# Wendison/FCL-taco2

Hardware: AMD Instinct MI355X
Metric: mel-frames/sec (FCL-taco2-S forward, batch=32, 80-mel) (higher is better)
Workload: dtype f32 via bf16x3-split MFMA operands, fp32 accumulate (max-abs 8e-6 on mel vs the reference; FCL_PRECISION=0 = exact fp32 MFMA)

## Files before the change

### fcl-taco2_amd/csrc/capi.hip

```cpp
#include <stdarg.h>
#include <stdlib.h>
#include <string.h>

#include <map>
#include <mutex>
#include <utility>
#include <vector>

#include "fcl_common.h"

namespace fcl {

static thread_local char g_err[512] = "";
static thread_local int g_gemm_mode = FCL_GEMM_F32;

void set_error(const char* fmt, ...) {
    va_list ap;
    va_start(ap, fmt);
    vsnprintf(g_err, sizeof(g_err), fmt, ap);
    va_end(ap);
}

int check_hip(hipError_t e, const char* what) {
    static const int sync_debug = getenv("FCL_SYNC_DEBUG") ? atoi(getenv("FCL_SYNC_DEBUG")) : 0;
// ... 474 lines not shown
    FCL_REQUIRE(io->dropout_mode != FCL_DROP_MASK || io->prenet_keep, FCL_ERR_INVALID, "decoder_loop_fwd: FCL_DROP_MASK needs prenet_keep");
    FCL_REQUIRE(w->prenet_dropout >= 0.f && w->prenet_dropout < 1.f, FCL_ERR_INVALID, "decoder_loop_fwd: bad prenet_dropout");
    FCL_REQUIRE(io->workspace && aligned16(io->workspace) && io->workspace_bytes >= fcl_decoder_loop_workspace_bytes(w, io->n), FCL_ERR_WORKSPACE,
                "decoder_loop_fwd: workspace missing, misaligned or smaller than fcl_decoder_loop_workspace_bytes()");
    FCL_REQUIRE(!io->live_rows || io->status, FCL_ERR_INVALID, "decoder_loop_fwd: device live_rows need a device status word");
    {
        int prev = io->n;
        FCL_REQUIRE(io->live_rows || io->live_rows_host[0] == io->n, FCL_ERR_INVALID, "decoder_loop_fwd: live_rows_host[0] must equal N (all durations > 0)");
        for (int t = 0; t < io->lmax; ++t) {
            FCL_REQUIRE(io->live_rows_host[t] > 0 && io->live_rows_host[t] <= prev, FCL_ERR_INVALID,
                        "decoder_loop_fwd: live_rows_host must be positive and non-increasing (rows sorted by duration descending)");
            prev = io->live_rows_host[t];
        }
    }
    hipStream_t s = (hipStream_t)stream;
    if (generic) return decoder_loop_generic(w, io, s);
    const int N = io->n, C = w->c, P = w->p, U = w->u, O = w->odim;
    DecoderWs ws = carve(w, N, io->workspace);

    static const bool planes_on = tunable("PRECISION", 1) != 0 && tunable("PLANES", 1) != 0;
    const bool planes = decoder_planes(w) && io->att_c_p != nullptr && planes_on;
    FCL_REQUIRE(planes || io->att_c, FCL_ERR_INVALID, "decoder_loop_fwd: att_c is required when the P32 path is off");
    FCL_REQUIRE(!io->before_p || planes, FCL_ERR_INVALID, "decoder_loop_fwd: before_p needs the P32 weight planes and att_c_p");
    {
        hipLaunchKernelGGL(zero_kernel, dim3(512), dim3(256), 0, s, ws.h0[0], (long long)(ws.state_bytes / 4));
        FCL_HIP(hipGetLastError());
    }
    const int ldc = C / 32, ldp = P / 32, ldu = U / 32;
    auto small_step = [&](int m) { return lstm_step_is_small(m, U); };
    {
        GemmArgs g = {};
        g.term[0] = GemmTerm{io->att_c, w->w0_att, C, C, C, 0};
        if (planes) { g.term[0].Ap = io->att_c_p; g.term[0].Wp = w->w0_att_p; g.term[0].lda_p = g.term[0].ldw_p = ldc; }
        g.nterms = 1; g.M = N; g.N = 4 * U; g.bias = w->b0; g.Y = ws.G0; g.ldy = 4 * U;
        int rc = launch_gemm(g, s);
        if (rc) return rc;
        GemmArgs f = {};
        f.term[0] = GemmTerm{io->att_c, w->wf_att, C, C, C, 0};
        if (planes) { f.term[0].Ap = io->att_c_p; f.term[0].Wp = w->wf_att_p; f.term[0].lda_p = f.term[0].ldw_p = ldc; }
        f.nterms = 1; f.M = N; f.N = O; f.Y = ws.F0; f.ldy = O;
        rc = launch_gemm(f, s);
        if (rc) return rc;
    }
    const float keep_scale = 1.0f / (1.0f - w->prenet_dropout);
    const int drop_mode = (w->prenet_dropout > 0.f) ? io->dropout_mode : FCL_DROP_NONE;
    {
        static const int tile_on = tunable("DEC_TILE", 0), tile_min = tunable("DEC_TILE_MIN_ROWS", 1024);
        if (tile_on && planes && w->stream && decoder_tile_shape_ok(w) && N >= tile_min && io->lmax <= 64 && !io->teacher_ys && !io->tap_prenet && !io->tap_lstm0 &&
            !io->tap_lstm1 && drop_mode != FCL_DROP_MASK && gemm_mode() != FCL_GEMM_BF16)
            return launch_decoder_tile(w, io, ws.G0, ws.F0, ws.c0, ws.c1, drop_mode, 0, nullptr, nullptr, s);
    }
    const bool tile_ok = planes && w->stream && decoder_tile_shape_ok(w) && io->lmax <= 64 && !io->teacher_ys && !io->tap_prenet && !io->tap_lstm0 && !io->tap_lstm1 &&
                         drop_mode != FCL_DROP_MASK && gemm_mode() != FCL_GEMM_BF16;
    const int tail_from = (tile_ok && io->tail_from > 0 && io->tail_from < io->lmax) ? io->tail_from : 0;
    int cur = 0;
    for (int t = 0; t <= io->lmax; ++t) {
        const bool hand_over = tail_from > 0 && t == tail_from;
        const int n = (t < io->lmax && !hand_over) ? io->live_rows_host[t] : 0;
        const int n_prev = t > 0 ? io->live_rows_host[t - 1] : 0;
        const uint8_t* keep0 = drop_mode == FCL_DROP_MASK && t < io->lmax ? io->prenet_keep + ((size_t)(t * 2 + 0) * N) * P : nullptr;
        const uint8_t* keep1 = drop_mode == FCL_DROP_MASK && t < io->lmax ? io->prenet_keep + ((size_t)(t * 2 + 1) * N) * P : nullptr;
        const unsigned seed0 = io->seed * 2654435761u + (unsigned)(t * 2 + 0), seed1 = seed0 + 1;
        const float* teacher_in = (io->teacher_ys && t > 0) ? io->teacher_ys + (size_t)(t - 1) * O : nullptr;
        FeatPrenetArgs fp = {};
        fp.M_feat = n_prev; fp.M_pre = n; fp.U = U; fp.O = O; fp.P = P;
        fp.h1 = t > 0 ? ws.h1[cur] : nullptr; fp.wf_h = w->wf_h; fp.F0 = ws.F0;
        fp.before = io->before; fp.frame_off = io->frame_off; fp.t_prev = t - 1; fp.t_cur = t;
        fp.teacher_in = teacher_in; fp.teacher_ld = io->lmax * O;
        if (t < io->lmax && !hand_over) { fp.w0 = w->prenet_w0; fp.b0 = w->prenet_b0; fp.w1 = w->prenet_w1; fp.b1 = w->prenet_b1; }
        fp.wf_hi = w->wf_h_hi; fp.wf_lo = w->wf_h_lo; fp.w0_hi = w->prenet_w0_hi; fp.w0_lo = w->prenet_w0_lo;
        fp.w1_hi = w->prenet_w1_hi; fp.w1_lo = w->prenet_w1_lo;
        fp.wf_ff = w->wf_h_ff; fp.w0_ff = w->prenet_w0_ff; fp.w1_ff = w->prenet_w1_ff;
        fp.drop_mode = drop_mode; fp.keep0 = keep0; fp.keep1 = keep1; fp.keep_scale = keep_scale; fp.drop_p = w->prenet_dropout;
        fp.seed0 = seed0; fp.seed1 = seed1; fp.seed_dev = io->seed_dev; fp.pre_out = ws.pre_b; fp.tap_prenet = io->tap_prenet;
        fp.live = io->live_rows; fp.status = io->status; fp.out_act = w->out_act;
        if (planes) {
            fp.before_p = io->before_p;
            if (!small_step(n)) { fp.pre_out_p = ws.pre_p; fp.pre_out = nullptr; }
        }
        int rc = launch_feat_prenet(fp, s);
        if (rc) return rc;
        if (hand_over) return launch_decoder_tile(w, io, ws.G0, ws.F0, ws.c0, ws.c1, drop_mode, t, ws.h0[cur], ws.h1[cur], s);
        if (t == io->lmax) break;
        LstmStepArgs l0 = {};
        const bool big = planes && !small_step(n);
        const bool next_big = planes && t + 1 < io->lmax && !small_step(io->live_rows_host[t + 1]);
        l0.term[0] = GemmTerm{ws.pre_b, w->w0_pre, P, P, P, 0, w->w0_pre_hi, w->w0_pre_lo};
        l0.term[1] = GemmTerm{ws.h0[cur], w->w0_hh, U, U, U, 0, w->w0_hh_hi, w->w0_hh_lo};
        if (big) {
            l0.term[0].Ap = ws.pre_p; l0.term[0].Wp = w->w0_pre_p; l0.term[0].lda_p = l0.term[0].ldw_p = ldp;
            l0.term[1].Ap = ws.h0_p[cur]; l0.term[1].Wp = w->w0_hh_p; l0.term[1].lda_p = l0.term[1].ldw_p = ldu;
            l0.h_out_p = ws.h0_p[cur ^ 1]; l0.ld_hp = ldu;
        }
        l0.term[0].Wff = w->w0_pre_ff; l0.term[1].Wff = w->w0_hh_ff;
        l0.nterms = 2; l0.M = n; l0.U = U; l0.G = ws.G0; l0.g_row_mul = 1; l0.g_row_add = 0;
        l0.m_dev = io->live_rows ? io->live_rows + t : nullptr;
        l0.rank1_w = w->w0_pos; l0.dur = io->dur; l0.step = t;
        l0.h_in = ws.h0[cur]; l0.h_out = ws.h0[cur ^ 1]; l0.c = ws.c0; l0.zoneout = w->zoneout_rate;
        if (io->tap_lstm0) { l0.out2 = io->tap_lstm0; l0.out2_row_base = io->frame_off; l0.out2_row_add = t; l0.ld2 = U; }
        rc = launch_lstm_step(l0, s);
        if (rc) return rc;
        LstmStepArgs l1 = {};
        l1.term[0] = GemmTerm{ws.h0[cur ^ 1], w->w1_ih, U, U, U, 0, w->w1_ih_hi, w->w1_ih_lo};
        l1.term[1] = GemmTerm{ws.h1[cur], w->w1_hh, U, U, U, 0, w->w1_hh_hi, w->w1_hh_lo};
        if (big) {
            l1.term[0].Ap = ws.h0_p[cur ^ 1]; l1.term[0].Wp = w->w1_ih_p; l1.term[0].lda_p = l1.term[0].ldw_p = ldu;
            l1.term[1].Ap = ws.h1_p[cur]; l1.term[1].Wp = w->w1_hh_p; l1.term[1].lda_p = l1.term[1].ldw_p = ldu;
            if (next_big) { l1.h_out_p = ws.h1_p[cur ^ 1]; l1.ld_hp = ldu; }
        }
        l1.term[0].Wff = w->w1_ih_ff; l1.term[1].Wff = w->w1_hh_ff;
        l1.nterms = 2; l1.M = n; l1.U = U; l1.bias = w->b1; l1.step = t;
        l1.m_dev = l0.m_dev;
        l1.h_in = ws.h1[cur]; l1.h_out = ws.h1[cur ^ 1]; l1.c = ws.c1; l1.zoneout = w->zoneout_rate;
        if (io->tap_lstm1) { l1.out2 = io->tap_lstm1; l1.out2_row_base = io->frame_off; l1.out2_row_add = t; l1.ld2 = U; }
        rc = launch_lstm_step(l1, s);
        if (rc) return rc;
        cur ^= 1;
    }
    return 0;
}

}
```

### fcl-taco2_amd/csrc/decoder_step.hip

```cpp
#include "fcl_common.h"
#include "lstm_epilogue.h"

namespace fcl {

typedef float f32x4 __attribute__((ext_vector_type(4)));

template <int NT>
__device__ __forceinline__ void rowtile_mma(const float* A_l, int lda_l, const float* const (&wrow)[NT], int K, int r16, int kq,
                                            f32x4 (&out)[NT], int rot = 0) {
    f32x4 acc0[NT], acc1[NT];
#pragma unroll
    for (int t = 0; t < NT; ++t) acc0[t] = acc1[t] = (f32x4){0.f, 0.f, 0.f, 0.f};
    const float* ap = A_l + r16 * lda_l + kq * 4;
    const float* wp[NT];
#pragma unroll
    for (int t = 0; t < NT; ++t) wp[t] = wrow[t] + kq * 4;
    const int nfull = K >> 6;
    f32x4 bn[NT][4];
    int cc = nfull > 0 ? rot % nfull : 0;
    if (nfull > 0) {
#pragma unroll
        for (int t = 0; t < NT; ++t)
#pragma unroll
            for (int i = 0; i < 4; ++i) bn[t][i] = *reinterpret_cast<const f32x4*>(wp[t] + (cc << 6) + i * 16);
// ... 848 lines not shown
        }
    }
}

template <bool PRE>
__global__ __launch_bounds__(256) void lstm_small_x3_kernel(const LstmStepArgs a) {
    const int M = a.M, Ms = live_rows_of(a.M, a.m_dev);
    if ((int)blockIdx.y * 16 >= Ms) return;
    constexpr int KC = 512;
    __shared__ __attribute__((aligned(16))) u16 A_h[16 * (KC + 16)];
    __shared__ __attribute__((aligned(16))) u16 A_lo[16 * (KC + 16)];
    __shared__ float g_l[4][16][17];
    const int m0 = blockIdx.y * 16, u0 = blockIdx.x * 16;
    const int lane = threadIdx.x & 63, g = threadIdx.x >> 6;
    const int r16 = lane & 15, kq = lane >> 4;
    const int erow = threadIdx.x >> 4, euc = threadIdx.x & 15;
    const int em = m0 + erow, eu = u0 + euc;
    const bool evalid = em < M && eu < a.U;
    CellIn ci;
    if (evalid) ci = cell_prefetch(a, em, eu);
    f32x4 acc = {0.f, 0.f, 0.f, 0.f};
    WFrag<1, 8> wf[2];
    if (PRE) {
#pragma unroll
        for (int t = 0; t < 2; ++t) {
            const size_t fo = (size_t)((g * a.U + u0) >> 4) * 8 * 512 + (size_t)lane * 8;
            const u16* const wh[1] = {a.term[t].Whi + fo};
            const u16* const wl[1] = {a.term[t].Wlo + fo};
            wf[t].load(wh, wl);
        }
#pragma unroll
        for (int t = 0; t < 2; ++t) {
            if (t) __syncthreads();
            load_rowtile_split(A_h, A_lo, 256 + 16, a.term[t].A, a.term[t].lda, 256, m0, M);
            __syncthreads();
            f32x4 part[1];
            wf[t].mma(A_h, A_lo, 256 + 16, 256, r16, kq, part);
            acc += part[0];
        }
    }
    for (int t = 0; t < (PRE ? 0 : a.nterms); ++t) {
        const GemmTerm T = a.term[t];
        for (int k0 = 0; k0 < T.K; k0 += KC) {
            const int kc = min(KC, T.K - k0);
            __syncthreads();
            load_rowtile_split(A_h, A_lo, kc + 16, T.A + k0, T.lda, kc, m0, M);
            __syncthreads();
            const size_t fo = ((size_t)((g * a.U + u0) >> 4) * ((T.K + 31) >> 5) + (k0 >> 5)) * 512 + (size_t)lane * 8;
            const u16* const wh[1] = {T.Whi + fo};
            const u16* const wl[1] = {T.Wlo + fo};
            f32x4 part[1];
            rowtile_mma_x3<1>(A_h, A_lo, kc + 16, wh, wl, kc, r16, kq, part);
            acc += part[0];
        }
    }
// ... 5 lines not shown
    __syncthreads();
    if (!evalid || em >= Ms) return;
    const float pre[4] = {g_l[0][erow][euc], g_l[1][erow][euc], g_l[2][erow][euc], g_l[3][erow][euc]};
    cell_finish(a, em, eu, pre, ci);
}


__global__ __launch_bounds__(256) void lstm_small_ff_kernel(const LstmStepArgs a) {
    const int M = a.M, Ms = live_rows_of(a.M, a.m_dev);
    if ((int)blockIdx.y * 16 >= Ms) return;
    constexpr int LD = 256 + 8;
    __shared__ __attribute__((aligned(16))) float A_f[16 * LD];
    __shared__ float g_l[4][16][17];
    const int m0 = blockIdx.y * 16, u0 = blockIdx.x * 16;
    const int lane = threadIdx.x & 63, g = threadIdx.x >> 6;
    const int r16 = lane & 15, kq = lane >> 4;
    const int erow = threadIdx.x >> 4, euc = threadIdx.x & 15;
    const int em = m0 + erow, eu = u0 + euc;
    const bool evalid = em < M && eu < a.U;
    CellIn ci;
    if (evalid) ci = cell_prefetch(a, em, eu);
    f32x4 acc = {0.f, 0.f, 0.f, 0.f};
    WFragF<1, 8> wf[2];
#pragma unroll
    for (int t = 0; t < 2; ++t) {
        const float* const w[1] = {a.term[t].Wff + (size_t)((g * a.U + u0) >> 4) * 8 * 512 + (size_t)lane * 8};
        wf[t].load(w);
    }
#pragma unroll
    for (int t = 0; t < 2; ++t) {
        if (t) __syncthreads();
        load_rowtile(A_f, LD, a.term[t].A, a.term[t].lda, 256, m0, M);
        __syncthreads();
        f32x4 part[1];
        mma_tf<1, 8>(wf[t], A_f, LD, r16, kq, part);
        acc += part[0];
    }
    {
        const int arow = lane & 15, cq = lane >> 4;
#pragma unroll
        for (int i = 0; i < 4; ++i) g_l[g][arow][cq * 4 + i] = acc[i];
    }
    __syncthreads();
    if (!evalid || em >= Ms) return;
    const float pre[4] = {g_l[0][erow][euc], g_l[1][erow][euc], g_l[2][erow][euc], g_l[3][erow][euc]};
    cell_finish(a, em, eu, pre, ci);
}

constexpr int SMALL_KC = 512;

__device__ __forceinline__ void lstm_small_body(const LstmStepArgs& a) {
    const int M = a.M, Ms = live_rows_of(a.M, a.m_dev);
    if ((int)blockIdx.y * 16 >= Ms) return;
// ... 25 lines not shown
    __syncthreads();
    const int row = threadIdx.x >> 4, uc = threadIdx.x & 15;
    const int m = m0 + row, uu = u0 + uc;
    if (m >= Ms || uu >= a.U) return;
    const CellIn ci = cell_prefetch(a, m, uu);
    const float pre[4] = {g_l[0][row][uc], g_l[1][row][uc], g_l[2][row][uc], g_l[3][row][uc]};
    cell_finish(a, m, uu, pre, ci);
}

__global__ __launch_bounds__(256) void lstm_small_kernel(const LstmStepArgs a) { lstm_small_body(a); }

__global__ __launch_bounds__(256) void lstm_small_pair_kernel(const LstmStepArgs a0, const LstmStepArgs a1) {
    if (blockIdx.z == 0) lstm_small_body(a0);
    else lstm_small_body(a1);
}

int launch_lstm_small(const LstmStepArgs& a, hipStream_t s) {
    double ksum = 0;
    for (int i = 0; i < a.nterms; ++i) ksum += a.term[i].K;
    dim3 grid((a.U + 15) / 16, (a.M + 15) / 16);
    bool planes = true;
    for (int i = 0; i < a.nterms; ++i) planes = planes && a.term[i].Whi && a.term[i].Wlo && (a.term[i].K & 7) == 0 && a.term[i].ldw == a.term[i].K;
    planes = planes && (a.U & 15) == 0;
    if (planes) {
        ProfScope ps("lstm_small_kernel/bf16x3", 2.0 * a.M * 4.0 * a.U * ksum, a.M, s);
        if (a.nterms == 2 && a.term[0].K == 256 && a.term[1].K == 256) hipLaunchKernelGGL(lstm_small_x3_kernel<true>, grid, dim3(256), 0, s, a);
        else hipLaunchKernelGGL(lstm_small_x3_kernel<false>, grid, dim3(256), 0, s, a);
    } else if (a.nterms == 2 && a.term[0].Wff && a.term[1].Wff && a.term[0].K == 256 && a.term[1].K == 256 && (a.U & 15) == 0) {
        ProfScope ps("lstm_small_ff_kernel/f32", 2.0 * a.M * 4.0 * a.U * ksum, a.M, s);
        hipLaunchKernelGGL(lstm_small_ff_kernel, grid, dim3(256), 0, s, a);
    } else {
        ProfScope ps("lstm_small_kernel", 2.0 * a.M * 4.0 * a.U * ksum, a.M, s);
        hipLaunchKernelGGL(lstm_small_kernel, grid, dim3(256), 0, s, a);
    }
    return check_hip(hipGetLastError(), "lstm_small launch");
}

int launch_lstm_small_pair(const LstmStepArgs& a0, const LstmStepArgs& a1, hipStream_t s) {
    double fl = 0;
    for (const LstmStepArgs* a : {&a0, &a1}) {
        double ksum = 0;
        for (int i = 0; i < a->nterms; ++i) ksum += a->term[i].K;
        fl += 2.0 * a->M * 4.0 * a->U * ksum;
    }
    const int mmax = a0.M > a1.M ? a0.M : a1.M;
    dim3 grid((a0.U + 15) / 16, (mmax + 15) / 16, 2);
    ProfScope ps("lstm_small_pair_kernel", fl, a0.M + a1.M, s);
    hipLaunchKernelGGL(lstm_small_pair_kernel, grid, dim3(256), 0, s, a0, a1);
    return check_hip(hipGetLastError(), "lstm_small_pair launch");
}

// ... 79 lines not shown
```

### fcl-taco2_amd/csrc/gemm_f32.hip

```cpp
#include <string.h>

#include "fcl_common.h"
#include "lstm_epilogue.h"

namespace fcl {

typedef float f32x4 __attribute__((ext_vector_type(4)));

#ifndef FCL_BK
#define FCL_BK 32
#endif
constexpr int BK = FCL_BK;
constexpr int F4 = BK / 4;
constexpr int F4_SHIFT = F4 == 8 ? 3 : 2;
static_assert(BK == 32 || BK == 16, "BK must be 16 or 32");
#ifndef FCL_NBUF
#define FCL_NBUF 2
#endif
constexpr int NBUF = FCL_NBUF;
constexpr int LDS_LD = BK + 4;

template <int WM, int WN, bool LSTM, int TM = 1>
struct Geo {
    static constexpr int BM = 16 * WM * TM;
// ... 389 lines not shown
    using G = Geo<WM, WN, false, TM>;
    dim3 grid((a.N + G::BN - 1) / G::BN, (a.M + G::BM - 1) / G::BM);
    char full[64];
    GemmArgs b = a;
    b.hi_only = precision() && gemm_mode() == FCL_GEMM_BF16;
    snprintf(full, sizeof(full), "gemm_kernel<%d,%d,%d,%d>%s", WM, WN, precision() ? 1 : 0, TM, b.hi_only ? "/bf16" : precision() ? "/bf16x3" : "");
    static const int shapes = tunable("PROF_SHAPES", 0);
    if (shapes && g_prof_on) {
        long long ks = 0;
        for (int i = 0; i < a.nterms; ++i) ks += a.term[i].K;
        const size_t l = strlen(full);
        snprintf(full + l, sizeof(full) - l, " %dx%dx%lld", a.M, a.N, ks);
    }
    (void)name;
    ProfScope ps(full, flops, a.M, s);
    if (precision()) hipLaunchKernelGGL((gemm_kernel<WM, WN, 1, TM>), grid, dim3(G::THREADS), 0, s, b);
    else hipLaunchKernelGGL((gemm_kernel<WM, WN, 0, TM>), grid, dim3(G::THREADS), 0, s, b);
}

template <int WM, int WN, int TM = 1>
static void launch_lstm_cfg(const LstmStepArgs& a, hipStream_t s, const char* name, double flops) {
    using G = Geo<WM, WN, true, TM>;
    dim3 grid((a.U + 16 * WN - 1) / (16 * WN), (a.M + G::BM - 1) / G::BM);
    const bool plain = !a.zone_keep_h && !a.row_len;
    const int mode = (plain && a.G && a.rank1_w && !a.bias) ? 0 : (plain && a.bias && !a.G && !a.rank1_w) ? 1 : -1;
    char full[64];
    const int hi_only = precision() && gemm_mode() == FCL_GEMM_BF16;
    snprintf(full, sizeof(full), "lstm_step_kernel<%d,%d,%d,%d,%d>%s", WM, WN, mode, precision() ? 1 : 0, TM, hi_only ? "/bf16" : precision() ? "/bf16x3" : "");
    (void)name;
    ProfScope ps(full, flops, a.M, s);
    if (precision()) {
        if (mode == 0) hipLaunchKernelGGL((lstm_step_kernel<WM, WN, 0, 1, TM>), grid, dim3(G::THREADS), 0, s, a, hi_only);
        else if (mode == 1) hipLaunchKernelGGL((lstm_step_kernel<WM, WN, 1, 1, TM>), grid, dim3(G::THREADS), 0, s, a, hi_only);
        else hipLaunchKernelGGL((lstm_step_kernel<WM, WN, -1, 1, TM>), grid, dim3(G::THREADS), 0, s, a, hi_only);
    } else {
        if (mode == 0) hipLaunchKernelGGL((lstm_step_kernel<WM, WN, 0, 0, TM>), grid, dim3(G::THREADS), 0, s, a, hi_only);
        else if (mode == 1) hipLaunchKernelGGL((lstm_step_kernel<WM, WN, 1, 0, TM>), grid, dim3(G::THREADS), 0, s, a, hi_only);
        else hipLaunchKernelGGL((lstm_step_kernel<WM, WN, -1, 0, TM>), grid, dim3(G::THREADS), 0, s, a, hi_only);
    }
}

extern thread_local bool t_exact_lines;
static bool exact_lines_ok(const GemmTerm* t, int n) {
    if (precision()) return false;
    for (int i = 0; i < n; ++i) {
        if (!t[i].A || !t[i].W || (t[i].K & 31) || (t[i].lda & 31) || (t[i].ldw & 31) || t[i].lda < t[i].K || t[i].ldw < t[i].K || t[i].a_chunk_stride) return false;
        if ((reinterpret_cast<uintptr_t>(t[i].A) | reinterpret_cast<uintptr_t>(t[i].W)) & 127u) return false;
// ... 77 lines not shown
    if (a.N >= 128 && (long long)((a.M + 63) / 64) * ((a.N + 127) / 128) >= tm2_min_wg()) {
        launch_gemm_cfg<2, 2, 2>(a, s, "gemm_kernel<2,2,tm2>", flops);
    } else if (a.M > 32) {
        launch_gemm_cfg<4, 1>(a, s, "gemm_kernel<4,1>", flops);
    } else if (a.M > 16) {
        launch_gemm_cfg<2, 2>(a, s, "gemm_kernel<2,2>", flops);
    } else {
        launch_gemm_cfg<1, 4>(a, s, "gemm_kernel<1,4>", flops);
    }
    return check_hip(hipGetLastError(), "gemm launch");
}

bool lstm_step_is_small(int M, int U) {
    static const int small_m = tunable("LSTM_SMALL_M", 0);
    static const bool planes_on = tunable("PRECISION", 1) == 0 || tunable("PLANES", 1) != 0;
    return M <= (small_m ? small_m : (U >= 512 ? (planes_on ? 64 : 256) : (planes_on ? 512 : 1024)));
}

int validate_lstm_step(const LstmStepArgs& a) {
    FCL_REQUIRE(a.M >= 0 && a.U > 0, FCL_ERR_SHAPE, "lstm_step: bad M=%d U=%d", a.M, a.U);
    if (a.M == 0) return 0;
    int rc = check_terms(a.term, a.nterms, 3, false, nullptr);
    if (rc) return rc;
    FCL_REQUIRE(a.h_in && a.h_out && a.c && a.h_in != a.h_out, FCL_ERR_INVALID, "lstm_step: h_in/h_out/c must be set and h_out must not alias h_in");
    FCL_REQUIRE(!a.rank1_w || a.dur, FCL_ERR_INVALID, "lstm_step: rank1_w needs dur");
    FCL_REQUIRE((a.zone_keep_h == nullptr) == (a.zone_keep_c == nullptr), FCL_ERR_INVALID, "lstm_step: zoneout masks come in pairs");
    return 0;
}
bool lstm_step_on_planes(const LstmStepArgs& a) { return precision() && planes_ok(a.term, a.nterms); }

int launch_lstm_step(const LstmStepArgs& a, hipStream_t s) {
    int rc = validate_lstm_step(a);
    if (rc) return rc;
    if (a.M == 0) return 0;
    const bool small = lstm_step_is_small(a.M, a.U);
    bool has_f32 = true;
    for (int i = 0; i < a.nterms; ++i) has_f32 = has_f32 && a.term[i].A && a.term[i].W;
    if (precision() && planes_ok(a.term, a.nterms) && (!small || !has_f32)) return launch_lstm_planes(a, s);
    FCL_REQUIRE(has_f32, FCL_ERR_INVALID, "lstm_step: the fp32-operand kernels need A and W of every term");
    if (small) return launch_lstm_small(a, s);
    if (!a.h_out_p && exact_lines_ok(a.term, a.nterms)) {
        LstmStepArgs b = a;
        exact_lines_terms(b, a.nterms);
        ExactScope sc;
        return launch_lstm_planes(b, s);
    }
    double ksum = 0;
// ... 17 lines not shown
```

### fcl-taco2_amd/csrc/gemm_planes.hip

```cpp
#include <string.h>

#include <type_traits>

#include "fcl_common.h"
#include "lstm_epilogue.h"

namespace fcl {

typedef float f32x4 __attribute__((ext_vector_type(4)));
typedef unsigned short u16;
typedef unsigned char u8;

__device__ __attribute__((aligned(128))) unsigned int g_zero_line[32];

typedef __attribute__((address_space(3))) void* lds_ptr_t;
typedef const __attribute__((address_space(1))) void* gbl_ptr_t;
__device__ __forceinline__ void glds16(const void* g, void* l) { __builtin_amdgcn_global_load_lds((gbl_ptr_t)g, (lds_ptr_t)l, 16, 0, 0); }

template <int N>
__device__ __forceinline__ void wait_vm() {
    asm volatile("s_waitcnt vmcnt(%0)" ::"n"(N) : "memory");
}

__constant__ int g_tile_group = 8;
// ... 67 lines not shown
#pragma unroll
    for (int tm = 0; tm < TM; ++tm) {
#pragma unroll
        for (int tn = 0; tn < TN; ++tn) acc[tm][tn] = __builtin_amdgcn_mfma_f32_16x16x32_bf16(al[tm], bh[tn], acc[tm][tn], 0, 0, 0);
#pragma unroll
        for (int tn = 0; tn < TN; ++tn) acc[tm][tn] = __builtin_amdgcn_mfma_f32_16x16x32_bf16(ah[tm], bl[tn], acc[tm][tn], 0, 0, 0);
#pragma unroll
        for (int tn = 0; tn < TN; ++tn) acc[tm][tn] = __builtin_amdgcn_mfma_f32_16x16x32_bf16(ah[tm], bh[tn], acc[tm][tn], 0, 0, 0);
    }
}

template <int WM, int WN, int TM, int TN, int NST, int LW = 0>
struct PGeo {
    static constexpr int BM = 16 * WM * TM, BN = 16 * WN * TN, NW = WM * WN, THREADS = 64 * (NW + LW), CTHREADS = 64 * NW;
    static constexpr int NL = LW > 0 ? LW : NW;
    static constexpr int GA = BM / 8 / NL, GB = BN / 8 / NL, GPW = GA + GB;
    static constexpr int STAGE = (BM + BN) * 128;
    static constexpr int LDS_BYTES = NST * STAGE;
    static_assert((BM / 8) % NL == 0 && (BN / 8) % NL == 0 && (NL % 2) == 0, "tile rows must split evenly over the loading waves");
    static_assert(NST >= 2 && NST <= 4, "ring depth (2: 64 KB for a 128 x 128 tile -> TWO workgroups per CU, one's epilogue beside the other's main loop)");
    static_assert(2 * GPW <= 60, "s_waitcnt vmcnt is a 6-bit field");
};

template <int WM, int WN, int TM, int TN, int NST, bool LSTM, int LW, int HI>
__device__ __forceinline__ bool pmainloop(const GemmTerm* __restrict__ terms, int nterms, int M, int m0, int n0, int NU, const int* __restrict__ seg_lo,
                                          const int* __restrict__ seg_hi, u8* smem, f32x4 (&acc)[TM][TN], int ksplit_chunks = 0) {
    using G = PGeo<WM, WN, TM, TN, NST, LW>;
    static_assert(!LSTM || TN == 4, "LSTM tiles keep the four gates of a unit in one lane");
    const int tid = threadIdx.x, lane = tid & 63;
    const int wave = __builtin_amdgcn_readfirstlane(tid >> 6);
    const bool loader = LW > 0 && wave >= G::NW;
    const int lw = LW > 0 ? wave - G::NW : wave;
    const int wm = wave / WN, wn = wave % WN;
    int nchunks = 0;
    for (int t = 0; t < nterms; ++t) nchunks += (terms[t].K + 31) >> 5;
    int kskip = 0;
    if (ksplit_chunks > 0) {
        kskip = (int)blockIdx.z * ksplit_chunks;
        nchunks = max(0, min(ksplit_chunks, nchunks - kskip));
    }

    if (LW == 0 || loader) {
        const unsigned coff = (unsigned)(((lane & 7) ^ (((lw & 1) << 2) | (lane >> 4))) * 16);
        const u8* zline = reinterpret_cast<const u8*>(g_zero_line) + coff;
        int am[G::GA], alo[G::GA];
        unsigned alen[G::GA];
#pragma unroll
        for (int j = 0; j < G::GA; ++j) {
            const int m = m0 + (j * G::NL + lw) * 8 + (lane >> 3);
            am[j] = m;
            alo[j] = 0;
            alen[j] = m < M ? (unsigned)M : 0u;
            if (seg_lo != nullptr && m < M) {
                alo[j] = seg_lo[m];
// ... 361 lines not shown
        for (int j = 0; j < TN; ++j) acc[i][j] = (f32x4){0.f, 0.f, 0.f, 0.f};
    if (!pmainloop<WM, WN, TM, TN, NST, false, LW, HI>(a.term, a.nterms, a.M, m0, n0, a.N, a.seg_lo, a.seg_hi, smem, acc, a.ksplit_chunks)) return;
    if (a.dbg_phase == 1) {
        float sdbg = 0.f;
#pragma unroll
        for (int i = 0; i < TM; ++i)
#pragma unroll
            for (int j = 0; j < TN; ++j) sdbg += (acc[i][j][0] + acc[i][j][1]) + (acc[i][j][2] + acc[i][j][3]);
        if (sdbg == 12345.678f) a.Y[0] = sdbg;
        return;
    }

    pgemm_epilogue<WN, TM, TN, G::BM, G::BN, G::CTHREADS, G::LDS_BYTES>(a, acc, smem, m0, n0);
}

template <int WM, int WN, int TM, int NST, int MODE, int LW, int HI>
__device__ __forceinline__ void plstm_body(const LstmStepArgs& a, u8* smem) {
    using G = PGeo<WM, WN, TM, 4, NST, LW>;
    int bx, by;
    xcd_tile_p(bx, by);
    const int m0 = by * G::BM, u0 = bx * (16 * WN);
    const int M = a.M, Ms = live_rows_of(a.M, a.m_dev);
    if (m0 >= Ms) return;
    const int lane = threadIdx.x & 63, wave = threadIdx.x >> 6;
    const int wm = wave / WN, wn = wave % WN;
    const int u = u0 + wn * 16 + (lane & 15);
    const int rq = lane >> 4;
    constexpr bool PRE = NST != 2;
    CellIn ci[PRE ? TM : 1][4];
    const int uc = min(u, a.U - 1);
    if (PRE && (LW == 0 || wave < G::NW)) {
#pragma unroll
        for (int tm = 0; tm < TM; ++tm)
#pragma unroll
            for (int r = 0; r < 4; ++r) ci[tm][r] = cell_prefetch<MODE>(a, min(m0 + (wm * TM + tm) * 16 + rq * 4 + r, M - 1), uc);
    }
    f32x4 acc[TM][4];
#pragma unroll
    for (int tm = 0; tm < TM; ++tm)
#pragma unroll
        for (int j = 0; j < 4; ++j) acc[tm][j] = (f32x4){0.f, 0.f, 0.f, 0.f};
    if (!pmainloop<WM, WN, TM, 4, NST, true, LW, HI>(a.term, a.nterms, M, m0, u0, a.U, nullptr, nullptr, smem, acc)) return;
    if (g_plstm_dbg == 1) {
        float sdbg = 0.f;
#pragma unroll
        for (int i = 0; i < TM; ++i)
#pragma unroll
            for (int j = 0; j < 4; ++j) sdbg += (acc[i][j][0] + acc[i][j][1]) + (acc[i][j][2] + acc[i][j][3]);
        if (sdbg == 12345.678f) a.h_out[0] = sdbg;
        return;
    }
    constexpr int UW = 16 * WN, LDT = UW + 4;
    static_assert(2 * G::BM * LDT * 4 <= G::LDS_BYTES, "the staging tiles must fit the ring");
    float* th = reinterpret_cast<float*>(smem);
    float* tc = th + G::BM * LDT;
    __syncthreads();
#pragma unroll
    for (int tm = 0; tm < TM; ++tm)
#pragma unroll
        for (int r = 0; r < 4; ++r) {
            const int rm = (wm * TM + tm) * 16 + rq * 4 + r, m = m0 + rm;
            float h_w = 0.f, c_w = 0.f;
            if (m < Ms && u < a.U) {
                const float pre[4] = {acc[tm][0][r], acc[tm][1][r], acc[tm][2][r], acc[tm][3][r]};
                if (PRE) {
                    cell_math<MODE>(a, m, u, pre, ci[PRE ? tm : 0][r], h_w, c_w);
                } else {
                    const CellIn cl = cell_prefetch<MODE>(a, m, u);
                    cell_math<MODE>(a, m, u, pre, cl, h_w, c_w);
                }
            }
            th[rm * LDT + wn * 16 + (lane & 15)] = h_w;
            tc[rm * LDT + wn * 16 + (lane & 15)] = c_w;
        }
    __syncthreads();
    const int rows = min(G::BM, Ms - m0);
    const bool vec = (a.U & 3) == 0;
    for (int i = threadIdx.x; i < rows * (UW / 4); i += G::CTHREADS) {
        const int rm = i / (UW / 4), c4 = (i - rm * (UW / 4)) * 4, uu = u0 + c4;
        if (uu >= a.U) continue;
        const f32x4 hv = *reinterpret_cast<const f32x4*>(th + rm * LDT + c4), cv = *reinterpret_cast<const f32x4*>(tc + rm * LDT + c4);
        const size_t off = (size_t)(m0 + rm) * a.U + uu;
        if (vec && uu + 3 < a.U) {
            *reinterpret_cast<f32x4*>(a.h_out + off) = hv;
            *reinterpret_cast<f32x4*>(a.c + off) = cv;
        } else {
#pragma unroll
            for (int e = 0; e < 4; ++e)
                if (uu + e < a.U) { a.h_out[off + e] = hv[e]; a.c[off + e] = cv[e]; }
        }
    }
    if (a.h_out_p) {
// ... 311 lines not shown
    const double flops = 2.0 * a.M * (double)a.N * ksum;
    const long long t64x128 = (long long)((a.M + 63) / 64) * ((a.N + 127) / 128);
    const long long t128x128 = (long long)((a.M + 127) / 128) * ((a.N + 127) / 128);
    if (!t_exact_lines && a.conv_k >= 3 && a.conv_k <= 17 && !a.accumulate && a.term[0].K <= 384) {
        static const int cbig_min = tunable("PCONV_BIG_MIN", 60);
        if (t128x128 >= cbig_min && a.N >= 128) return launch_pconv_cfg<4, 2, 2, 4>(a, s, flops);
        if (t64x128 >= 250 && a.N >= 96) return launch_pconv_cfg<2, 2, 2, 4>(a, s, flops);
        return launch_pconv_cfg<2, 2, 2, 2>(a, s, flops);
    }
    if (a.accumulate)
        return (a.M >= 128 && a.N >= 128) ? launch_pgemm_cfg<4, 2, 2, 4, 3>(a, s, flops) : launch_pgemm_cfg<2, 2, 2, 2, 4>(a, s, flops);
    static const int two_stage_min = tunable("PGEMM_2STAGE_MIN_WG", 300);
    if (t128x128 >= two_stage_min && a.N >= 256) return launch_pgemm_cfg<4, 2, 2, 4, 2>(a, s, flops);
    static const int gbig_min = tunable("PGEMM_BIG_MIN", 150);
    if (t128x128 >= gbig_min && a.N >= 128) return launch_pgemm_cfg<4, 2, 2, 4, 3>(a, s, flops);
    if (t64x128 >= 250 && a.N >= 96) return launch_pgemm_cfg<2, 2, 2, 4, 3>(a, s, flops);
    return launch_pgemm_cfg<2, 2, 2, 2, 4>(a, s, flops);
}

template <int WM, int WN, int TM, int NST, int LW, int HI>
static int launch_plstm_lw(const LstmStepArgs& a, hipStream_t s, double flops) {
    using G = PGeo<WM, WN, TM, 4, NST, LW>;
    const bool plain = !a.zone_keep_h && !a.row_len && !a.save_gates && !a.out2;
    const int mode = (plain && a.G && a.rank1_w && !a.bias) ? 0 : (plain && a.bias && !a.G && !a.rank1_w) ? 1 : -1;
    dim3 grid((a.U + 16 * WN - 1) / (16 * WN), (a.M + G::BM - 1) / G::BM);
    char full[64];
    snprintf(full, sizeof(full), "plstm_kernel<%d,%d,%d,%d,%d,%d>%s", WM, WN, TM, NST, mode, LW, HI == 2 ? "/f32" : HI ? "/bf16" : "");
    const void* fn = mode == 0 ? reinterpret_cast<const void*>(plstm_kernel<WM, WN, TM, NST, 0, LW, HI>)
                   : mode == 1 ? reinterpret_cast<const void*>(plstm_kernel<WM, WN, TM, NST, 1, LW, HI>)
                               : reinterpret_cast<const void*>(plstm_kernel<WM, WN, TM, NST, -1, LW, HI>);
    const int rc = ensure_dyn_lds(fn, G::LDS_BYTES);
    if (rc) return rc;
    double fill = 0.0;
    {
        long long nch = 0;
        for (int i = 0; i < a.nterms; ++i) nch += (a.term[i].K + 31) >> 5;
        fill = (double)grid.x * grid.y * (double)nch * (G::BM + G::BN) * 128.0;
    }
    ProfScope ps(full, flops, a.M, s, fill);
    if (mode == 0) hipLaunchKernelGGL((plstm_kernel<WM, WN, TM, NST, 0, LW, HI>), grid, dim3(G::THREADS), G::LDS_BYTES, s, a);
    else if (mode == 1) hipLaunchKernelGGL((plstm_kernel<WM, WN, TM, NST, 1, LW, HI>), grid, dim3(G::THREADS), G::LDS_BYTES, s, a);
    else hipLaunchKernelGGL((plstm_kernel<WM, WN, TM, NST, -1, LW, HI>), grid, dim3(G::THREADS), G::LDS_BYTES, s, a);
    return check_hip(hipGetLastError(), "plstm launch");
}

template <int WM, int WN, int TM, int NST>
static int launch_plstm_cfg(const LstmStepArgs& a, hipStream_t s, double flops) {
    if (t_exact_lines) return launch_plstm_lw<WM, WN, TM, NST, 4, 2>(a, s, flops);
    if (gemm_mode() == FCL_GEMM_BF16) return launch_plstm_lw<WM, WN, TM, NST, 2, true>(a, s, flops);
    return launch_plstm_lw<WM, WN, TM, NST, 4, false>(a, s, flops);
}

int launch_lstm_planes(const LstmStepArgs& a, hipStream_t s) {
    FCL_REQUIRE(!a.h_out_p || ((a.U & 31) == 0 && a.ld_hp * 32 >= a.U && (reinterpret_cast<uintptr_t>(a.h_out_p) & 127u) == 0), FCL_ERR_SHAPE,
                "lstm_step: h_out_p needs U %% 32 == 0, ld_hp >= U / 32 and a 128-byte aligned buffer");
    double ksum = 0;
    for (int i = 0; i < a.nterms; ++i) ksum += a.term[i].K;
    const double flops = 2.0 * a.M * 4.0 * a.U * ksum;
    const long long t128 = (long long)((a.M + 127) / 128) * ((a.U + 31) / 32);
    const long long t64 = (long long)((a.M + 63) / 64) * ((a.U + 31) / 32);
    static const int two_stage_min = tunable("PLSTM_2STAGE_MIN_WG", 125);
    static const int two_stage_min_exact = tunable("PLSTM_2STAGE_MIN_WG_EXACT", 300);
    if (t128 >= (t_exact_lines ? two_stage_min_exact : two_stage_min) && !a.zone_keep_h && !a.save_gates) return launch_plstm_cfg<4, 2, 2, 2>(a, s, flops);
    static const int big_min_t = tunable("PLSTM_BIG_MIN", 150), big_min_s = tunable("PLSTM_BIG_MIN_S", 300);
    static const int mid_min_t = tunable("PLSTM_MID_MIN", 200), mid_min_s = tunable("PLSTM_MID_MIN_S", 80);
// ... 817 lines not shown
```

### fcl-taco2_amd/csrc/lstm_epilogue.h

```cpp
#pragma once
#include "fcl_common.h"

namespace fcl {

__device__ __forceinline__ float sigmoid_f(float x) { return __builtin_amdgcn_rcpf(1.0f + __expf(-x)); }
__device__ __forceinline__ float tanh_f(float x) { return 1.0f - 2.0f * __builtin_amdgcn_rcpf(1.0f + __expf(2.0f * x)); }
__device__ __forceinline__ float act_apply(float v, int act) {
    return act == FCL_ACT_RELU ? fmaxf(v, 0.f) : (act == FCL_ACT_TANH ? tanh_f(v) : (act == FCL_ACT_SIGMOID ? sigmoid_f(v) : v));
}

struct CellIn {
    float add[4];
    float h_old, c_old;
    bool live;
};

template <int MODE = -1>
__device__ __forceinline__ CellIn cell_prefetch(const LstmStepArgs& a, int m, int u) {
    CellIn ci;
    const bool has_bias = MODE < 0 ? a.bias != nullptr : MODE == 1;
    const bool has_g = MODE < 0 ? a.G != nullptr : MODE == 0;
    const bool has_pos = MODE < 0 ? a.rank1_w != nullptr : MODE == 0;
#pragma unroll
    for (int g = 0; g < 4; ++g) ci.add[g] = has_bias ? a.bias[g * a.U + u] : 0.f;
    if (has_g) {
        const float* gr = a.G + (size_t)((long long)m * a.g_row_mul + a.g_row_add) * (4 * a.U);
#pragma unroll
        for (int g = 0; g < 4; ++g) ci.add[g] += gr[g * a.U + u];
    }
    if (has_pos) {
        const float pos = (float)a.step / (float)a.dur[m];
#pragma unroll
        for (int g = 0; g < 4; ++g) ci.add[g] += pos * a.rank1_w[g * a.U + u];
    }
    const size_t off = (size_t)m * a.U + u;
    ci.h_old = a.h_in[off];
    ci.c_old = a.c[off];
    ci.live = a.row_len ? (a.step < a.row_len[m]) : true;
    return ci;
}

template <int MODE = -1>
__device__ __forceinline__ void cell_math(const LstmStepArgs& a, int m, int u, const float (&acc)[4], const CellIn& ci, float& h_w, float& c_w) {
    const float ig = sigmoid_f(acc[0] + ci.add[0]), fg = sigmoid_f(acc[1] + ci.add[1]);
    const float gg = tanh_f(acc[2] + ci.add[2]), og = sigmoid_f(acc[3] + ci.add[3]);
    const float c_new = fg * ci.c_old + ig * gg;
    const float h_new = og * tanh_f(c_new);
    const size_t off = (size_t)m * a.U + u;
    float h_o, c_o;
    if (MODE < 0 && a.zone_keep_h) {
        h_o = a.zone_keep_h[off] ? ci.h_old : h_new;
        c_o = a.zone_keep_c[off] ? ci.c_old : c_new;
    } else {
        h_o = a.zoneout * ci.h_old + (1.0f - a.zoneout) * h_new;
        c_o = a.zoneout * ci.c_old + (1.0f - a.zoneout) * c_new;
    }
    if (MODE >= 0) {
        h_w = h_o;
        c_w = c_o;
        return;
    }
    h_w = ci.live ? h_o : ci.h_old;
    c_w = ci.live ? c_o : ci.c_old;
    if (a.save_gates) {
        float* sg = a.save_gates + (size_t)m * 4 * a.U;
        sg[u] = ig; sg[a.U + u] = fg; sg[2 * a.U + u] = gg; sg[3 * a.U + u] = og;
        a.save_c_new[off] = c_new;
        a.save_c_old[off] = ci.c_old;
// ... 19 lines not shown
```

Baseline: 48.40 million.

## Skip zero-state recurrent term at first decoder step and seed accumulators with bias

At decoder step 0 the LSTM hidden and cell states are known to be zero, so the recurrent GEMM term is dropped (nterms=1, h_in=nullptr) and the state reads are replaced by zeros. This removes the upfront state-zeroing kernel on the step-by-step path. New plstm kernel modes 2 and 3 cover the zero-state case. The LSTM kernel now initialises its accumulators with bias, G and position terms instead of adding them in the epilogue, and loader waves split off early through a fixed-role pmainloop. The gain is limited to one step out of many, and the extra template instantiations and added branches add complexity.

```diff
diff --git a/fcl-taco2_amd/csrc/capi.hip b/fcl-taco2_amd/csrc/capi.hip
--- a/fcl-taco2_amd/csrc/capi.hip
+++ b/fcl-taco2_amd/csrc/capi.hip
@@ -520,10 +520,6 @@
     const bool planes = decoder_planes(w) && io->att_c_p != nullptr && planes_on;
     FCL_REQUIRE(planes || io->att_c, FCL_ERR_INVALID, "decoder_loop_fwd: att_c is required when the P32 path is off");
     FCL_REQUIRE(!io->before_p || planes, FCL_ERR_INVALID, "decoder_loop_fwd: before_p needs the P32 weight planes and att_c_p");
-    {
-        hipLaunchKernelGGL(zero_kernel, dim3(512), dim3(256), 0, s, ws.h0[0], (long long)(ws.state_bytes / 4));
-        FCL_HIP(hipGetLastError());
-    }
     const int ldc = C / 32, ldp = P / 32, ldu = U / 32;
     auto small_step = [&](int m) { return lstm_step_is_small(m, U); };
     {
@@ -545,8 +541,11 @@
     {
         static const int tile_on = tunable("DEC_TILE", 0), tile_min = tunable("DEC_TILE_MIN_ROWS", 1024);
         if (tile_on && planes && w->stream && decoder_tile_shape_ok(w) && N >= tile_min && io->lmax <= 64 && !io->teacher_ys && !io->tap_prenet && !io->tap_lstm0 &&
-            !io->tap_lstm1 && drop_mode != FCL_DROP_MASK && gemm_mode() != FCL_GEMM_BF16)
+            !io->tap_lstm1 && drop_mode != FCL_DROP_MASK && gemm_mode() != FCL_GEMM_BF16) {
+            hipLaunchKernelGGL(zero_kernel, dim3(512), dim3(256), 0, s, ws.c0, (long long)((ws.c1 - ws.c0) + (size_t)N * U));
+            FCL_HIP(hipGetLastError());
             return launch_decoder_tile(w, io, ws.G0, ws.F0, ws.c0, ws.c1, drop_mode, 0, nullptr, nullptr, s);
+        }
     }
     const bool tile_ok = planes && w->stream && decoder_tile_shape_ok(w) && io->lmax <= 64 && !io->teacher_ys && !io->tap_prenet && !io->tap_lstm0 && !io->tap_lstm1 &&
                          drop_mode != FCL_DROP_MASK && gemm_mode() != FCL_GEMM_BF16;
@@ -591,10 +590,10 @@
             l0.h_out_p = ws.h0_p[cur ^ 1]; l0.ld_hp = ldu;
         }
         l0.term[0].Wff = w->w0_pre_ff; l0.term[1].Wff = w->w0_hh_ff;
-        l0.nterms = 2; l0.M = n; l0.U = U; l0.G = ws.G0; l0.g_row_mul = 1; l0.g_row_add = 0;
+        l0.nterms = t == 0 ? 1 : 2; l0.M = n; l0.U = U; l0.G = ws.G0; l0.g_row_mul = 1; l0.g_row_add = 0;
         l0.m_dev = io->live_rows ? io->live_rows + t : nullptr;
         l0.rank1_w = w->w0_pos; l0.dur = io->dur; l0.step = t;
-        l0.h_in = ws.h0[cur]; l0.h_out = ws.h0[cur ^ 1]; l0.c = ws.c0; l0.zoneout = w->zoneout_rate;
+        l0.h_in = t == 0 ? nullptr : ws.h0[cur]; l0.h_out = ws.h0[cur ^ 1]; l0.c = ws.c0; l0.zoneout = w->zoneout_rate;
         if (io->tap_lstm0) { l0.out2 = io->tap_lstm0; l0.out2_row_base = io->frame_off; l0.out2_row_add = t; l0.ld2 = U; }
         rc = launch_lstm_step(l0, s);
         if (rc) return rc;
@@ -607,9 +606,9 @@
             if (next_big) { l1.h_out_p = ws.h1_p[cur ^ 1]; l1.ld_hp = ldu; }
         }
         l1.term[0].Wff = w->w1_ih_ff; l1.term[1].Wff = w->w1_hh_ff;
-        l1.nterms = 2; l1.M = n; l1.U = U; l1.bias = w->b1; l1.step = t;
+        l1.nterms = t == 0 ? 1 : 2; l1.M = n; l1.U = U; l1.bias = w->b1; l1.step = t;
         l1.m_dev = l0.m_dev;
-        l1.h_in = ws.h1[cur]; l1.h_out = ws.h1[cur ^ 1]; l1.c = ws.c1; l1.zoneout = w->zoneout_rate;
+        l1.h_in = t == 0 ? nullptr : ws.h1[cur]; l1.h_out = ws.h1[cur ^ 1]; l1.c = ws.c1; l1.zoneout = w->zoneout_rate;
         if (io->tap_lstm1) { l1.out2 = io->tap_lstm1; l1.out2_row_base = io->frame_off; l1.out2_row_add = t; l1.ld2 = U; }
         rc = launch_lstm_step(l1, s);
         if (rc) return rc;
diff --git a/fcl-taco2_amd/csrc/decoder_step.hip b/fcl-taco2_amd/csrc/decoder_step.hip
--- a/fcl-taco2_amd/csrc/decoder_step.hip
+++ b/fcl-taco2_amd/csrc/decoder_step.hip
@@ -894,8 +894,10 @@
     f32x4 acc = {0.f, 0.f, 0.f, 0.f};
     WFrag<1, 8> wf[2];
     if (PRE) {
+        const int nt = a.nterms;
 #pragma unroll
         for (int t = 0; t < 2; ++t) {
+            if (t >= nt) break;
             const size_t fo = (size_t)((g * a.U + u0) >> 4) * 8 * 512 + (size_t)lane * 8;
             const u16* const wh[1] = {a.term[t].Whi + fo};
             const u16* const wl[1] = {a.term[t].Wlo + fo};
@@ -903,6 +905,7 @@
         }
 #pragma unroll
         for (int t = 0; t < 2; ++t) {
+            if (t >= nt) break;
             if (t) __syncthreads();
             load_rowtile_split(A_h, A_lo, 256 + 16, a.term[t].A, a.term[t].lda, 256, m0, M);
             __syncthreads();
@@ -954,13 +957,16 @@
     if (evalid) ci = cell_prefetch(a, em, eu);
     f32x4 acc = {0.f, 0.f, 0.f, 0.f};
     WFragF<1, 8> wf[2];
+    const int nt = a.nterms;
 #pragma unroll
     for (int t = 0; t < 2; ++t) {
+        if (t >= nt) break;
         const float* const w[1] = {a.term[t].Wff + (size_t)((g * a.U + u0) >> 4) * 8 * 512 + (size_t)lane * 8};
         wf[t].load(w);
     }
 #pragma unroll
     for (int t = 0; t < 2; ++t) {
+        if (t >= nt) break;
         if (t) __syncthreads();
         load_rowtile(A_f, LD, a.term[t].A, a.term[t].lda, 256, m0, M);
         __syncthreads();
@@ -1032,11 +1038,16 @@
     bool planes = true;
     for (int i = 0; i < a.nterms; ++i) planes = planes && a.term[i].Whi && a.term[i].Wlo && (a.term[i].K & 7) == 0 && a.term[i].ldw == a.term[i].K;
     planes = planes && (a.U & 15) == 0;
+    bool pre256 = a.nterms == 2 || (a.nterms == 1 && !a.h_in), ff = true;
+    for (int i = 0; i < a.nterms; ++i) {
+        pre256 = pre256 && a.term[i].K == 256;
+        ff = ff && a.term[i].Wff != nullptr;
+    }
     if (planes) {
         ProfScope ps("lstm_small_kernel/bf16x3", 2.0 * a.M * 4.0 * a.U * ksum, a.M, s);
-        if (a.nterms == 2 && a.term[0].K == 256 && a.term[1].K == 256) hipLaunchKernelGGL(lstm_small_x3_kernel<true>, grid, dim3(256), 0, s, a);
+        if (pre256) hipLaunchKernelGGL(lstm_small_x3_kernel<true>, grid, dim3(256), 0, s, a);
         else hipLaunchKernelGGL(lstm_small_x3_kernel<false>, grid, dim3(256), 0, s, a);
-    } else if (a.nterms == 2 && a.term[0].Wff && a.term[1].Wff && a.term[0].K == 256 && a.term[1].K == 256 && (a.U & 15) == 0) {
+    } else if (pre256 && ff && (a.U & 15) == 0) {
         ProfScope ps("lstm_small_ff_kernel/f32", 2.0 * a.M * 4.0 * a.U * ksum, a.M, s);
         hipLaunchKernelGGL(lstm_small_ff_kernel, grid, dim3(256), 0, s, a);
     } else {
diff --git a/fcl-taco2_amd/csrc/gemm_f32.hip b/fcl-taco2_amd/csrc/gemm_f32.hip
--- a/fcl-taco2_amd/csrc/gemm_f32.hip
+++ b/fcl-taco2_amd/csrc/gemm_f32.hip
@@ -435,7 +435,7 @@
 static void launch_lstm_cfg(const LstmStepArgs& a, hipStream_t s, const char* name, double flops) {
     using G = Geo<WM, WN, true, TM>;
     dim3 grid((a.U + 16 * WN - 1) / (16 * WN), (a.M + G::BM - 1) / G::BM);
-    const bool plain = !a.zone_keep_h && !a.row_len;
+    const bool plain = !a.zone_keep_h && !a.row_len && a.h_in;
     const int mode = (plain && a.G && a.rank1_w && !a.bias) ? 0 : (plain && a.bias && !a.G && !a.rank1_w) ? 1 : -1;
     char full[64];
     const int hi_only = precision() && gemm_mode() == FCL_GEMM_BF16;
@@ -559,7 +559,7 @@
     if (a.M == 0) return 0;
     int rc = check_terms(a.term, a.nterms, 3, false, nullptr);
     if (rc) return rc;
-    FCL_REQUIRE(a.h_in && a.h_out && a.c && a.h_in != a.h_out, FCL_ERR_INVALID, "lstm_step: h_in/h_out/c must be set and h_out must not alias h_in");
+    FCL_REQUIRE(a.h_out && a.c && a.h_in != a.h_out, FCL_ERR_INVALID, "lstm_step: h_out/c must be set and h_out must not alias h_in");
     FCL_REQUIRE(!a.rank1_w || a.dur, FCL_ERR_INVALID, "lstm_step: rank1_w needs dur");
     FCL_REQUIRE((a.zone_keep_h == nullptr) == (a.zone_keep_c == nullptr), FCL_ERR_INVALID, "lstm_step: zoneout masks come in pairs");
     return 0;
diff --git a/fcl-taco2_amd/csrc/gemm_planes.hip b/fcl-taco2_amd/csrc/gemm_planes.hip
--- a/fcl-taco2_amd/csrc/gemm_planes.hip
+++ b/fcl-taco2_amd/csrc/gemm_planes.hip
@@ -113,14 +113,15 @@
     static_assert(2 * GPW <= 60, "s_waitcnt vmcnt is a 6-bit field");
 };
 
-template <int WM, int WN, int TM, int TN, int NST, bool LSTM, int LW, int HI>
+template <int WM, int WN, int TM, int TN, int NST, bool LSTM, int LW, int HI, int ROLE = 0>
 __device__ __forceinline__ bool pmainloop(const GemmTerm* __restrict__ terms, int nterms, int M, int m0, int n0, int NU, const int* __restrict__ seg_lo,
                                           const int* __restrict__ seg_hi, u8* smem, f32x4 (&acc)[TM][TN], int ksplit_chunks = 0) {
     using G = PGeo<WM, WN, TM, TN, NST, LW>;
     static_assert(!LSTM || TN == 4, "LSTM tiles keep the four gates of a unit in one lane");
     const int tid = threadIdx.x, lane = tid & 63;
     const int wave = __builtin_amdgcn_readfirstlane(tid >> 6);
-    const bool loader = LW > 0 && wave >= G::NW;
+    static_assert(ROLE == 0 || LW > 0, "a role is fixed only where loader waves exist");
+    const bool loader = ROLE == 1 || (ROLE == 0 && LW > 0 && wave >= G::NW);
     const int lw = LW > 0 ? wave - G::NW : wave;
     const int wm = wave / WN, wn = wave % WN;
     int nchunks = 0;
@@ -528,25 +529,42 @@
     const int m0 = by * G::BM, u0 = bx * (16 * WN);
     const int M = a.M, Ms = live_rows_of(a.M, a.m_dev);
     if (m0 >= Ms) return;
-    const int lane = threadIdx.x & 63, wave = threadIdx.x >> 6;
+    const int lane = threadIdx.x & 63, wave = __builtin_amdgcn_readfirstlane(threadIdx.x >> 6);
+    f32x4 acc[TM][4];
+    if (LW > 0 && wave >= G::NW) {
+        (void)pmainloop<WM, WN, TM, 4, NST, true, LW, HI, 1>(a.term, a.nterms, M, m0, u0, a.U, nullptr, nullptr, smem, acc);
+        return;
+    }
     const int wm = wave / WN, wn = wave % WN;
     const int u = u0 + wn * 16 + (lane & 15);
     const int rq = lane >> 4;
+    constexpr bool SEED = MODE >= 0;
     constexpr bool PRE = NST != 2;
     CellIn ci[PRE ? TM : 1][4];
     const int uc = min(u, a.U - 1);
-    if (PRE && (LW == 0 || wave < G::NW)) {
+    if (PRE) {
 #pragma unroll
         for (int tm = 0; tm < TM; ++tm)
 #pragma unroll
-            for (int r = 0; r < 4; ++r) ci[tm][r] = cell_prefetch<MODE>(a, min(m0 + (wm * TM + tm) * 16 + rq * 4 + r, M - 1), uc);
-    }
-    f32x4 acc[TM][4];
+            for (int r = 0; r < 4; ++r) ci[tm][r] = cell_prefetch<MODE, SEED>(a, min(m0 + (wm * TM + tm) * 16 + rq * 4 + r, M - 1), uc);
+    }
 #pragma unroll
     for (int tm = 0; tm < TM; ++tm)
 #pragma unroll
         for (int j = 0; j < 4; ++j) acc[tm][j] = (f32x4){0.f, 0.f, 0.f, 0.f};
-    if (!pmainloop<WM, WN, TM, 4, NST, true, LW, HI>(a.term, a.nterms, M, m0, u0, a.U, nullptr, nullptr, smem, acc)) return;
+    if (SEED) {
+#pragma unroll
+        for (int tm = 0; tm < TM; ++tm)
+#pragma unroll
+            for (int r = 0; r < 4; ++r) {
+                const int mc = min(m0 + (wm * TM + tm) * 16 + rq * 4 + r, M - 1);
+                float add[4];
+                cell_seed<MODE>(a, mc, uc, cell_pos<MODE>(a, mc), add);
+#pragma unroll
+                for (int j = 0; j < 4; ++j) acc[tm][j][r] = add[j];
+            }
+    }
+    (void)pmainloop<WM, WN, TM, 4, NST, true, LW, HI, (LW > 0 ? 2 : 0)>(a.term, a.nterms, M, m0, u0, a.U, nullptr, nullptr, smem, acc);
     if (g_plstm_dbg == 1) {
         float sdbg = 0.f;
 #pragma unroll
@@ -570,10 +588,10 @@
             if (m < Ms && u < a.U) {
                 const float pre[4] = {acc[tm][0][r], acc[tm][1][r], acc[tm][2][r], acc[tm][3][r]};
                 if (PRE) {
-                    cell_math<MODE>(a, m, u, pre, ci[PRE ? tm : 0][r], h_w, c_w);
+                    cell_math<MODE, SEED>(a, m, u, pre, ci[PRE ? tm : 0][r], h_w, c_w);
                 } else {
-                    const CellIn cl = cell_prefetch<MODE>(a, m, u);
-                    cell_math<MODE>(a, m, u, pre, cl, h_w, c_w);
+                    const CellIn cl = cell_prefetch<MODE, SEED>(a, m, u);
+                    cell_math<MODE, SEED>(a, m, u, pre, cl, h_w, c_w);
                 }
             }
             th[rm * LDT + wn * 16 + (lane & 15)] = h_w;
@@ -931,14 +949,17 @@
 static int launch_plstm_lw(const LstmStepArgs& a, hipStream_t s, double flops) {
     using G = PGeo<WM, WN, TM, 4, NST, LW>;
     const bool plain = !a.zone_keep_h && !a.row_len && !a.save_gates && !a.out2;
-    const int mode = (plain && a.G && a.rank1_w && !a.bias) ? 0 : (plain && a.bias && !a.G && !a.rank1_w) ? 1 : -1;
+    const int layer = (plain && a.G && a.rank1_w && !a.bias) ? 0 : (plain && a.bias && !a.G && !a.rank1_w) ? 1 : -1;
+    const int mode = layer < 0 ? -1 : layer + (a.h_in ? 0 : 2);
     dim3 grid((a.U + 16 * WN - 1) / (16 * WN), (a.M + G::BM - 1) / G::BM);
     char full[64];
     snprintf(full, sizeof(full), "plstm_kernel<%d,%d,%d,%d,%d,%d>%s", WM, WN, TM, NST, mode, LW, HI == 2 ? "/f32" : HI ? "/bf16" : "");
-    const void* fn = mode == 0 ? reinterpret_cast<const void*>(plstm_kernel<WM, WN, TM, NST, 0, LW, HI>)
-                   : mode == 1 ? reinterpret_cast<const void*>(plstm_kernel<WM, WN, TM, NST, 1, LW, HI>)
-                               : reinterpret_cast<const void*>(plstm_kernel<WM, WN, TM, NST, -1, LW, HI>);
-    const int rc = ensure_dyn_lds(fn, G::LDS_BYTES);
+    void (*const fn)(const LstmStepArgs) = mode == 0   ? plstm_kernel<WM, WN, TM, NST, 0, LW, HI>
+                                           : mode == 1 ? plstm_kernel<WM, WN, TM, NST, 1, LW, HI>
+                                           : mode == 2 ? plstm_kernel<WM, WN, TM, NST, 2, LW, HI>
+                                           : mode == 3 ? plstm_kernel<WM, WN, TM, NST, 3, LW, HI>
+                                                       : plstm_kernel<WM, WN, TM, NST, -1, LW, HI>;
+    const int rc = ensure_dyn_lds(reinterpret_cast<const void*>(fn), G::LDS_BYTES);
     if (rc) return rc;
     double fill = 0.0;
     {
@@ -947,9 +968,7 @@
         fill = (double)grid.x * grid.y * (double)nch * (G::BM + G::BN) * 128.0;
     }
     ProfScope ps(full, flops, a.M, s, fill);
-    if (mode == 0) hipLaunchKernelGGL((plstm_kernel<WM, WN, TM, NST, 0, LW, HI>), grid, dim3(G::THREADS), G::LDS_BYTES, s, a);
-    else if (mode == 1) hipLaunchKernelGGL((plstm_kernel<WM, WN, TM, NST, 1, LW, HI>), grid, dim3(G::THREADS), G::LDS_BYTES, s, a);
-    else hipLaunchKernelGGL((plstm_kernel<WM, WN, TM, NST, -1, LW, HI>), grid, dim3(G::THREADS), G::LDS_BYTES, s, a);
+    hipLaunchKernelGGL(fn, grid, dim3(G::THREADS), G::LDS_BYTES, s, a);
     return check_hip(hipGetLastError(), "plstm launch");
 }
 
diff --git a/fcl-taco2_amd/csrc/lstm_epilogue.h b/fcl-taco2_amd/csrc/lstm_epilogue.h
--- a/fcl-taco2_amd/csrc/lstm_epilogue.h
+++ b/fcl-taco2_amd/csrc/lstm_epilogue.h
@@ -15,35 +15,55 @@
     bool live;
 };
 
+__host__ __device__ constexpr bool mode_layer0(int MODE) { return MODE == 0 || MODE == 2; }
+__host__ __device__ constexpr bool mode_layer1(int MODE) { return MODE == 1 || MODE == 3; }
+
 template <int MODE = -1>
+__device__ __forceinline__ float cell_pos(const LstmStepArgs& a, int m) {
+    const bool has_pos = MODE < 0 ? a.rank1_w != nullptr : mode_layer0(MODE);
+    return has_pos ? (float)a.step / (float)a.dur[m] : 0.f;
+}
+
+template <int MODE = -1>
+__device__ __forceinline__ void cell_seed(const LstmStepArgs& a, int m, int u, float pos, float (&add)[4]) {
+    const bool has_bias = MODE < 0 ? a.bias != nullptr : mode_layer1(MODE);
+    const bool has_g = MODE < 0 ? a.G != nullptr : mode_layer0(MODE);
+    const bool has_pos = MODE < 0 ? a.rank1_w != nullptr : mode_layer0(MODE);
+    if (MODE >= 0) {
+        const float* gr = has_g ? a.G + (size_t)((long long)m * a.g_row_mul + a.g_row_add) * (4 * a.U) : a.bias;
+#pragma unroll
+        for (int g = 0; g < 4; ++g) add[g] = gr[g * a.U + u];
+    } else {
+#pragma unroll
+        for (int g = 0; g < 4; ++g) add[g] = has_bias ? a.bias[g * a.U + u] : 0.f;
+        if (has_g) {
+            const float* gr = a.G + (size_t)((long long)m * a.g_row_mul + a.g_row_add) * (4 * a.U);
+#pragma unroll
+            for (int g = 0; g < 4; ++g) add[g] += gr[g * a.U + u];
+        }
+    }
+    if (has_pos) {
+#pragma unroll
+        for (int g = 0; g < 4; ++g) add[g] += pos * a.rank1_w[g * a.U + u];
+    }
+}
+
+template <int MODE = -1, bool SEEDED = false>
 __device__ __forceinline__ CellIn cell_prefetch(const LstmStepArgs& a, int m, int u) {
     CellIn ci;
-    const bool has_bias = MODE < 0 ? a.bias != nullptr : MODE == 1;
-    const bool has_g = MODE < 0 ? a.G != nullptr : MODE == 0;
-    const bool has_pos = MODE < 0 ? a.rank1_w != nullptr : MODE == 0;
-#pragma unroll
-    for (int g = 0; g < 4; ++g) ci.add[g] = has_bias ? a.bias[g * a.U + u] : 0.f;
-    if (has_g) {
-        const float* gr = a.G + (size_t)((long long)m * a.g_row_mul + a.g_row_add) * (4 * a.U);
-#pragma unroll
-        for (int g = 0; g < 4; ++g) ci.add[g] += gr[g * a.U + u];
-    }
-    if (has_pos) {
-        const float pos = (float)a.step / (float)a.dur[m];
-#pragma unroll
-        for (int g = 0; g < 4; ++g) ci.add[g] += pos * a.rank1_w[g * a.U + u];
-    }
+    if (!SEEDED) cell_seed<MODE>(a, m, u, cell_pos<MODE>(a, m), ci.add);
+    const bool zero_state = MODE < 0 ? a.h_in == nullptr : MODE >= 2;
     const size_t off = (size_t)m * a.U + u;
-    ci.h_old = a.h_in[off];
-    ci.c_old = a.c[off];
+    ci.h_old = zero_state ? 0.f : a.h_in[off];
+    ci.c_old = zero_state ? 0.f : a.c[off];
     ci.live = a.row_len ? (a.step < a.row_len[m]) : true;
     return ci;
 }
 
-template <int MODE = -1>
+template <int MODE = -1, bool SEEDED = false>
 __device__ __forceinline__ void cell_math(const LstmStepArgs& a, int m, int u, const float (&acc)[4], const CellIn& ci, float& h_w, float& c_w) {
-    const float ig = sigmoid_f(acc[0] + ci.add[0]), fg = sigmoid_f(acc[1] + ci.add[1]);
-    const float gg = tanh_f(acc[2] + ci.add[2]), og = sigmoid_f(acc[3] + ci.add[3]);
+    const float ig = sigmoid_f(SEEDED ? acc[0] : acc[0] + ci.add[0]), fg = sigmoid_f(SEEDED ? acc[1] : acc[1] + ci.add[1]);
+    const float gg = tanh_f(SEEDED ? acc[2] : acc[2] + ci.add[2]), og = sigmoid_f(SEEDED ? acc[3] : acc[3] + ci.add[3]);
     const float c_new = fg * ci.c_old + ig * gg;
     const float h_new = og * tanh_f(c_new);
     const size_t off = (size_t)m * a.U + u;
```

Result: faster. 49.76 million (median of 6 runs) (+2.8%).
